# nju-ee/MODE-2022

Hardware: AMD Instinct MI355X
Metric: ERP stereo pairs/sec (512x1024, 192 disp) fwd+bwd (higher is better)
Workload: dtype fp32 storage/accumulate; products: 2xfp16 split (22-bit, per-tensor 2^k scale, 3 MFMAs) in the stride-1 3x3x3 / spherical / 3x3 layers incl. gradients (DESIGN 3u/3v); 3xbf16 split (24-bit, 6 MFMAs) in the stride-2 / transposed 3x3x3 layers and the polar spherical tiles (3j-3l); fp32 MFMA in the 32->; 1 GPU; ModeDisparity(192,Sphere,1024x512 Cassini) fwd+bwd+Adam step, batch 2/GPU (BASELINE configs[2]); global_batch=2, conv_arith=bf16x6, init=recipe state, seed 1 (tests/golden/recipe.py), parallelism=dp1

## Files before the change

### mode-2022_amd/csrc/sphere_conv_win.hip

```cpp
#include <algorithm>
#include <cstring>
#include <vector>

#include "common.h"
#include "bn_internal.h"
#include "sphere_internal.h"
#include "sphere_tap.h"

namespace {

typedef float f32x16 __attribute__((ext_vector_type(16)));
typedef float f32x32 __attribute__((ext_vector_type(32)));

constexpr int RB = 2;
constexpr int TH = 32 * RB;
constexpr int TW = 4;
constexpr int WC = 8;
constexpr int CCH = 8;
constexpr int KT = 9;
constexpr int MTW = 4;
constexpr int NTHREADS = 64 * TW * RB;
constexpr int SROWS = NTHREADS / WC;
constexpr int WR_SMALL = TH + 17, WR_MID = TH + 81;
constexpr int WR_PIPE_MAX = 5 * SROWS;

struct WinDims {
  int B, Ci, H, W, Co, G;
  int Cig, Cog;
  int NCH;
  int MG;
  int wr;
  int wrap_pipe;
  int sh, sw;
  int accumulate;
};

__host__ __device__ constexpr int chan_pitch(int wr) {
  return WC * wr + ((32 - (WC * wr) % 64) + 64) % 64;
}

__device__ __forceinline__ f32x16 mfma32(float a, float b, f32x16 c) {
  return __builtin_amdgcn_mfma_f32_32x32x2f32(a, b, c, 0, 0, 0);
}

__global__ void pack_w_win(const float* __restrict__ w, float* __restrict__ wp, WinDims d, int fold, mode_bn_epilogue bn) {
  const long long total = (long long)d.G * d.MG * d.NCH * KT * MTW * 64 * 4;
  if (fold && blockIdx.x == 0)
    for (int o = threadIdx.x; o < d.Co; o += blockDim.x) wp[total + o] = fold_shift(bn, o);
  for (long long idx = (long long)blockIdx.x * blockDim.x + threadIdx.x; idx < total; idx += (long long)gridDim.x * blockDim.x) {
    const int s = (int)(idx & 3);
    const int lane = (int)((idx >> 2) & 63);
    long long r = idx >> 8;
    const int m = (int)(r % MTW);
    r /= MTW;
    const int tap = (int)(r % KT);
    r /= KT;
    const int ch = (int)(r % d.NCH);
    r /= d.NCH;
    const int mg = (int)(r % d.MG);
    const int g = (int)(r / d.MG);
    const int co = mg * 128 + m * 32 + (lane & 31);
    const int c = ch * CCH + 2 * s + (lane >> 5);
    float v = 0.f;
    if (co < d.Cog && c < d.Cig) {
      v = w[((long long)(g * d.Cog + co) * d.Cig + c) * KT + tap];
      if (fold) v *= fold_scale(bn, g * d.Cog + co);
    }
    wp[idx] = v;
  }
}

template <int WR_T, bool PIPE, int NRB, int NPH, bool EPI>
__device__ __forceinline__ void fwd_tile(const float* __restrict__ x, const float* __restrict__ pos, const float4* __restrict__ wp,
                                         float* __restrict__ y, const WinDims& d, int h0, int w0, int rbase, int cbase, float* smem,
                                         const Epi& epi) {
  const int WRP = WR_T > 0 ? WR_T : d.wr;
  const int CP = chan_pitch(WRP);
  const int bufsz = CCH * CP;

  const int b = blockIdx.y;
  const int g = blockIdx.z / d.MG, mg = blockIdx.z % d.MG;
  const int tid = threadIdx.x;
  const int wave = tid >> 6, lane = tid & 63;
  const int half = lane >> 5;
  const int h = h0 + (wave / TW) * 32 + (lane & 31), w = w0 + (wave % TW);
  const bool pix_ok = h < d.H && w < d.W;
  const long long HW = (long long)d.H * d.W;

// ... 168 lines not shown
          for (int r = 0; r < 16; ++r) {
            const int co = min(m * 32 + (r & 3) + 8 * (r >> 2) + 4 * half, cmax - 1);
            res[r] = epi.add[(yb - y) + (long long)co * HW];
          }
        }
        __builtin_amdgcn_sched_barrier(0);
      }
      auto emit = [&](int r) {
        const int co = m * 32 + (r & 3) + 8 * (r >> 2) + 4 * half;
        if (EPI) {
          const float v = (acc[m][r] + shv[r]) + res[r];
          yb[(long long)co * HW] = epi.relu ? relu_nan(v) : v;
        } else {
          yb[(long long)co * HW] = acc[m][r];
        }
      };
      if (m * 32 + 32 <= cmax) {
#pragma unroll
        for (int r = 0; r < 16; ++r) emit(r);
      } else {
#pragma unroll
        for (int r = 0; r < 16; ++r)
          if (m * 32 + (r & 3) + 8 * (r >> 2) + 4 * half < cmax) emit(r);
      }
      if (EPI) __builtin_amdgcn_sched_barrier(0);
    }
  }
}

template <bool EPI>
__global__ __launch_bounds__(NTHREADS) void sphere_fwd_win_kernel(const float* __restrict__ x, const float* __restrict__ pos,
                                                                   const float4* __restrict__ wp, float* __restrict__ y, WinDims d,
                                                                   const int4* __restrict__ tiles, Epi epi) {
  extern __shared__ __attribute__((aligned(16))) float smem[];
  const int4 t = tiles[blockIdx.x];
  const int cls = t.w >> 16, cbase = t.w & 0xffff;
  if (cls == 0)
    fwd_tile<WR_SMALL, true, (WR_SMALL + SROWS - 1) / SROWS, 1, EPI>(x, pos, wp, y, d, t.x, t.y, t.z, cbase, smem, epi);
  else if (cls == 1)
    fwd_tile<WR_MID, true, (WR_MID + SROWS - 1) / SROWS, 2, EPI>(x, pos, wp, y, d, t.x, t.y, t.z, cbase, smem, epi);
  else
    fwd_tile<0, true, WR_PIPE_MAX / SROWS, 4, EPI>(x, pos, wp, y, d, t.x, t.y, t.z, cbase, smem, epi);
}

template <bool EPI>
__global__ __launch_bounds__(NTHREADS) void sphere_fwd_win_tall_kernel(const float* __restrict__ x, const float* __restrict__ pos,
                                                                        const float4* __restrict__ wp, float* __restrict__ y,
                                                                        WinDims d, const int4* __restrict__ tiles, Epi epi) {
  extern __shared__ __attribute__((aligned(16))) float smem[];
  const int4 t = tiles[blockIdx.x];
  fwd_tile<0, false, 1, 1, EPI>(x, pos, wp, y, d, t.x, t.y, t.z, t.w & 0xffff, smem, epi);
}

constexpr int BW_CG = 32;
constexpr int BW_TH = 32;
constexpr int BW_WR = BW_TH + 17;
constexpr int BW_CP = WC * BW_WR + 1;
constexpr int BW_GP = BW_TH + 1;
constexpr int BW_SLOTS = KT;
constexpr int BW_XW = BW_CG * BW_CP + BW_WR + 8;
constexpr int BW_COLBUF = 128 * BW_GP;
constexpr int BW_LDS_FLOATS = 2 * BW_XW + 2 * BW_COLBUF;
constexpr int BW_NXW = BW_CG / TW;
constexpr int BW_NREC = KT * BW_TH;

template <int WRP, int CP>
__device__ __forceinline__ void bww_column(const float* cb, const float* xw, const float4 rw, const int ro, const float4 rw8,
                                           const int ro8, f32x32 (&accp)[2], f32x32 (&acc8p)[2], int wave_u, int j, int half) {
  const float* ap = cb + (half * 32 + j) * BW_GP;
  const float* xb = xw + j * CP;
  auto load_x = [&](int o, float (&raw)[4]) {
    const float* p = xb + o;
    raw[0] = p[0];
    raw[1] = p[WRP];
    raw[2] = p[1];
    raw[3] = p[WRP + 1];
  };
  auto bcast = [&](float v, int px) { return __builtin_bit_cast(float, __builtin_amdgcn_readlane(__builtin_bit_cast(int, v), px)); };
  auto combine = [&](const float4& w, int px, const float (&raw)[4]) {
    return __builtin_fmaf(bcast(w.w, px), raw[3],
                          __builtin_fmaf(bcast(w.z, px), raw[2], __builtin_fmaf(bcast(w.y, px), raw[1], bcast(w.x, px) * raw[0])));
  };
  {
    float raw[2][4], a[3][2];
#pragma unroll
    for (int p0 = 0; p0 < 2; ++p0) {
      load_x(__builtin_amdgcn_readlane(ro, p0), raw[p0]);
      a[p0][0] = ap[p0];
      a[p0][1] = ap[64 * BW_GP + p0];
    }
    float bv = combine(rw, 0, raw[0]);
#pragma unroll
    for (int px = 0; px < BW_TH; ++px) {
      const int c3 = px % 3, n3 = (px + 2) % 3;
      float bv_next = 0.f;
      if (px + 1 < BW_TH) bv_next = combine(rw, px + 1, raw[(px + 1) & 1]);
      if (px + 2 < BW_TH) {
        load_x(__builtin_amdgcn_readlane(ro, px + 2), raw[px & 1]);
        a[n3][0] = ap[px + 2];
        a[n3][1] = ap[64 * BW_GP + px + 2];
      }
      __builtin_amdgcn_sched_barrier(0);
      accp[0] = __builtin_amdgcn_mfma_f32_32x32x1f32(a[c3][0], bv, accp[0], 0, 0, 0);
      accp[1] = __builtin_amdgcn_mfma_f32_32x32x1f32(a[c3][1], bv, accp[1], 0, 0, 0);
      __builtin_amdgcn_sched_barrier(0);
      bv = bv_next;
    }
  }
  {
    float raw[4][4], a[4][2];
#pragma unroll
    for (int i = 0; i < BW_TH / 8; ++i) {
      const int px = wave_u + 8 * i;
      load_x(__builtin_amdgcn_readlane(ro8, px), raw[i]);
      a[i][0] = ap[px];
      a[i][1] = ap[64 * BW_GP + px];
    }
// ... 272 lines not shown
    const float* pp = part + ((((long long)z * NCG + cg) * BW_SLOTS + k) * 128 + row) * BW_CG + cl;
    float a0 = 0.f, a1 = 0.f, a2 = 0.f, a3 = 0.f;
    int e = 0;
    for (; e + 3 < S; e += 4) {
      a0 += pp[(long long)e * stride];
      a1 += pp[(long long)(e + 1) * stride];
      a2 += pp[(long long)(e + 2) * stride];
      a3 += pp[(long long)(e + 3) * stride];
    }
    for (; e < S; ++e) a0 += pp[(long long)e * stride];
    const float sum = (a0 + a1) + (a2 + a3);
    gw[((long long)(g * d.Cog + ol) * d.Cig + c) * KT + k] += sum;
  }
}

bool halves_fit(const float* pos_host, int H, int W, int KK, int h0, int w0, int rbase, int cbase) {
  const long long HW = (long long)H * W;
  for (int hf = 0; hf < 2; ++hf) {
    const int rb = (rbase + hf * BW_TH) % H;
    for (int k = 0; k < KK; ++k)
      for (int h = h0 + hf * BW_TH; h < std::min(h0 + (hf + 1) * BW_TH, H); ++h)
        for (int w = w0; w < std::min(w0 + TW, W); ++w) {
          int r0, c0;
          float4 wt;
          const long long idx = (long long)h * W + w;
          if (!mode::tap_record_fixed(pos_host[(2 * k) * HW + idx], pos_host[(2 * k + 1) * HW + idx], H, W, r0, c0, wt)) continue;
          if (wt.x == 0.f && wt.y == 0.f && wt.z == 0.f && wt.w == 0.f) continue;
          const int lr = ((r0 - rb) % H + H) % H;
          if (lr + 1 >= BW_WR || c0 - cbase < 0 || c0 - cbase + 1 >= WC) return false;
        }
  }
  return true;
}

int bww_win_splits(const WinDims& d, int ntiles) {
  const int T = ntiles * 2 * d.B;
  const int wgs_per_slice = mode::cdiv(d.Cig, BW_CG) * d.G * d.MG;
  const int per = std::max(1, mode::cdiv((long long)T * wgs_per_slice, kNumCU));
  return std::max(1, mode::cdiv(T, per));
}


constexpr int SP_CCH = 16;
constexpr int SP_CP = chan_pitch(WR_SMALL);
constexpr int SP_WIN = SP_CCH * SP_CP;
constexpr int SP_WIN_FLOATS = ((2 * SP_WIN + WR_SMALL + 8 + 3) / 4) * 4;
constexpr int SP_OP = 8 * 3 * 64;
constexpr size_t SP_LDS_BYTES = (size_t)SP_WIN_FLOATS * sizeof(float) + 2 * (size_t)SP_OP * sizeof(uint4);
constexpr size_t SP3_LDS_BYTES = SP_LDS_BYTES + (size_t)SP_OP * sizeof(uint4);
static_assert(SP3_LDS_BYTES <= 160 * 1024, "windows + three operand buffers must fit the 160 KB of a CU");

typedef __bf16 sp_bf16x8 __attribute__((ext_vector_type(8)));
typedef __bf16 sp_bf16x2 __attribute__((ext_vector_type(2)));
typedef float sp_f32x2 __attribute__((ext_vector_type(2)));

__device__ __forceinline__ uint32_t sp_pack2(float a, float b) {
  const sp_f32x2 v = {a, b};
  return __builtin_bit_cast(uint32_t, __builtin_convertvector(v, sp_bf16x2));
}
__device__ __forceinline__ void sp_split2(float a, float b, uint32_t& p1, uint32_t& p2, uint32_t& p3) {
  p1 = sp_pack2(a, b);
  float ra = a - __builtin_bit_cast(float, p1 << 16), rb = b - __builtin_bit_cast(float, p1 & 0xffff0000u);
  asm("" : "+v"(ra), "+v"(rb));
  p2 = sp_pack2(ra, rb);
  float sa = ra - __builtin_bit_cast(float, p2 << 16), sb = rb - __builtin_bit_cast(float, p2 & 0xffff0000u);
  asm("" : "+v"(sa), "+v"(sb));
  p3 = sp_pack2(sa, sb);
}
__device__ __forceinline__ f32x16 sp_mfma(uint4 a, uint4 b, f32x16 c) {
  return __builtin_amdgcn_mfma_f32_32x32x16_bf16(__builtin_bit_cast(sp_bf16x8, a), __builtin_bit_cast(sp_bf16x8, b), c, 0, 0, 0);
}
__device__ __forceinline__ void sp_lds_barrier() { asm volatile("s_waitcnt lgkmcnt(0)\n\ts_barrier" ::: "memory"); }

typedef _Float16 sp_f16x2 __attribute__((ext_vector_type(2)));
typedef _Float16 sp_f16x8 __attribute__((ext_vector_type(8)));
__device__ __forceinline__ float sp_f16_scale_of(float m) {
  const unsigned e = min(max((__builtin_bit_cast(unsigned, m) >> 23) & 0xffu, 64u), 254u);
  return m == 0.f ? 1.f : __builtin_bit_cast(float, (268u - e) << 23);
}
__device__ __forceinline__ void sp_split2_f16(float a, float b, uint32_t& p1, uint32_t& p2) {
  const sp_f32x2 v = {a, b};
  const sp_f16x2 h1 = __builtin_convertvector(v, sp_f16x2);
  p1 = __builtin_bit_cast(uint32_t, h1);
  float ra, rb;
  asm("v_fma_mix_f32 %0, 1.0, %3, -%2 op_sel_hi:[0,0,1]\n\t"
      "v_fma_mix_f32 %1, 1.0, %4, -%2 op_sel:[0,0,1] op_sel_hi:[0,0,1]"
      : "=&v"(ra), "=&v"(rb)
      : "v"(p1), "v"(a), "v"(b));
  const sp_f32x2 r = {ra, rb};
  p2 = __builtin_bit_cast(uint32_t, __builtin_convertvector(r, sp_f16x2));
}
__device__ __forceinline__ f32x16 sp_mfma_f16(uint4 a, uint4 b, f32x16 c) {
  return __builtin_amdgcn_mfma_f32_32x32x16_f16(__builtin_bit_cast(sp_f16x8, a), __builtin_bit_cast(sp_f16x8, b), c, 0, 0, 0);
}

template <bool F16>
__global__ void pack_w_win_split(const float* __restrict__ w, uint4* __restrict__ wps, WinDims d, int NCH16, int fold, mode_bn_epilogue bn,
                                 const float* __restrict__ amax_w) {
  const float sw = F16 ? sp_f16_scale_of(mode::absmax_load(amax_w)) : 1.f;
  const long long total = (long long)d.G * d.MG * NCH16 * KT * MTW * 64;
  for (long long idx = (long long)blockIdx.x * blockDim.x + threadIdx.x; idx < total; idx += (long long)gridDim.x * blockDim.x) {
    const int lane = (int)(idx & 63);
    long long r = idx >> 6;
    const int m = (int)(r % MTW);
    r /= MTW;
    const int tap = (int)(r % KT);
    r /= KT;
    const int ch = (int)(r % NCH16);
    r /= NCH16;
    const int mg = (int)(r % d.MG);
    const int g = (int)(r / d.MG);
    const int co = mg * 128 + m * 32 + (lane & 31);
    float v[8];
#pragma unroll
    for (int j = 0; j < 8; ++j) {
      const int c = ch * SP_CCH + 8 * (lane >> 5) + j;
      v[j] = 0.f;
      if (co < d.Cog && c < d.Cig) {
        v[j] = w[((long long)(g * d.Cog + co) * d.Cig + c) * KT + tap];
        if (fold) v[j] *= fold_scale(bn, g * d.Cog + co);
        if (F16) v[j] *= sw;
      }
    }
    uint32_t q1[4], q2[4], q3[4];
#pragma unroll
    for (int j = 0; j < 4; ++j) {
      if constexpr (F16) {
        sp_split2_f16(v[2 * j], v[2 * j + 1], q1[j], q2[j]);
        q3[j] = 0u;
      } else {
        sp_split2(v[2 * j], v[2 * j + 1], q1[j], q2[j], q3[j]);
      }
    }
    uint4* dst = wps + (idx - lane) * 3 + lane;
    dst[0] = make_uint4(q1[0], q1[1], q1[2], q1[3]);
    dst[64] = make_uint4(q2[0], q2[1], q2[2], q2[3]);
    dst[128] = make_uint4(q3[0], q3[1], q3[2], q3[3]);
  }
}

constexpr int TP = 5;

template <bool F16>
__global__ void pack_w_win_split_tall(const float* __restrict__ w, uint4* __restrict__ wpt, WinDims d, int fold, mode_bn_epilogue bn,
                                      const float* __restrict__ amax_w) {
  const float sw = F16 ? sp_f16_scale_of(mode::absmax_load(amax_w)) : 1.f;
  const long long total = (long long)d.G * d.MG * d.NCH * TP * MTW * 64;
// ... 811 lines not shown
  }
#undef MODE_SB
  MODE_STAMP(2)

  const int hh = h0 + (wave / TW) * 32 + (lane & 31);
  const int cmax = d.Cog - mg * 128;
  float shv[16];
  if (EPI) {
#pragma unroll
    for (int r = 0; r < 16; ++r) shv[r] = epi.shift[g * d.Cog + mg * 128 + min(m * 32 + (r & 3) + 8 * (r >> 2) + 4 * half, cmax - 1)];
  }
  const bool full_m = m * 32 + 32 <= cmax;
#pragma unroll
  for (int gi = 0; gi < 4; ++gi) {
    const int ww = w0 + gi;
    if (hh < d.H && ww < d.W) {
      float* yb = y + ((long long)b * d.Co + (long long)g * d.Cog + (long long)mg * 128) * HW + (long long)hh * d.sh + (long long)ww * d.sw;
      float res[16];
      if (EPI) {
#pragma unroll
        for (int r = 0; r < 16; ++r) res[r] = 0.f;
        if (epi.add) {
#pragma unroll
          for (int r = 0; r < 16; ++r) {
            const int co = min(m * 32 + (r & 3) + 8 * (r >> 2) + 4 * half, cmax - 1);
            res[r] = epi.add[(yb - y) + (long long)co * HW];
          }
        }
        __builtin_amdgcn_sched_barrier(0);
      }
      auto emit = [&](int r) {
        const int co = m * 32 + (r & 3) + 8 * (r >> 2) + 4 * half;
        if (EPI) {
          const float v = (acc[gi][r] + shv[r]) + res[r];
          yb[(long long)co * HW] = epi.relu ? relu_nan(v) : v;
        } else {
          yb[(long long)co * HW] = F16 ? acc[gi][r] * unscale : acc[gi][r];
        }
      };
      if (full_m) {
#pragma unroll
        for (int r = 0; r < 16; ++r) emit(r);
      } else {
#pragma unroll
        for (int r = 0; r < 16; ++r)
          if (m * 32 + (r & 3) + 8 * (r >> 2) + 4 * half < cmax) emit(r);
      }
      if (EPI) __builtin_amdgcn_sched_barrier(0);
    }
  }
  MODE_STAMP(3)
}

constexpr int BS_GP = 20;
constexpr int BS_GYB = 3 * 128 * BS_GP;
constexpr int BS_SCRP = 17;
constexpr int BS_SCR = 32 * BS_SCRP;
constexpr int BS_X2 = ((2 * BW_XW + 3) / 4) * 4;
constexpr int BS_LDS_DWORDS = BS_X2 + BS_GYB + 8 * BS_SCR;

template <bool F16>
__global__ __launch_bounds__(NTHREADS) void sphere_bww_split_kernel(const float* __restrict__ gy, const float* __restrict__ x,
                                                                     float* __restrict__ part, WinDims d, const int4* __restrict__ tiles,
                                                                     const float4* __restrict__ rec_w, const int* __restrict__ rec_off,
                                                                     int ntiles, int S, const float* __restrict__ amax_g,
                                                                     const float* __restrict__ amax_x) {
  extern __shared__ __attribute__((aligned(16))) float smem[];
  float sg = 1.f, sx = 1.f, unscale = 1.f;
  if (F16) {
    sg = sp_f16_scale_of(mode::absmax_load(amax_g));
    sx = sp_f16_scale_of(mode::absmax_load(amax_x));
    unscale = (1.f / sg) * (1.f / sx);
  }
  constexpr int NPC = F16 ? 2 : 3;
  uint32_t* gyb = reinterpret_cast<uint32_t*>(smem + BS_X2);
  constexpr int WRP = BW_WR, CP = BW_CP;
  const int s = blockIdx.x, cg = blockIdx.y;
  const int g = blockIdx.z / d.MG, mg = blockIdx.z % d.MG;
  const int tid = threadIdx.x;
  const int wave = tid >> 6, lane = tid & 63;
  const int j = lane & 31, half = lane >> 5;
  float* scr = smem + BS_X2 + BS_GYB + wave * BS_SCR;
  const long long HW = (long long)d.H * d.W;
  const int T = ntiles * 2 * d.B;
  const int NCG = gridDim.y;

  f32x16 acc[4], acc8;
#pragma unroll
  for (int r = 0; r < 16; ++r) {
    acc[0][r] = acc[1][r] = acc[2][r] = acc[3][r] = 0.f;
    acc8[r] = 0.f;
  }
  for (int i = tid; i < BS_LDS_DWORDS; i += NTHREADS) smem[i] = 0.f;

  const int omax = d.Cog - mg * 128;
  const int cmax = d.Cig - cg * BW_CG;
  const int sh = half, sq = j >> 3, sp8 = j & 7;
  const int ks8 = wave >> 2, m8 = wave & 3;

  struct Item {
    int b, ti, hf, h0, w0, rbase, cbase;
  };
  auto item_of = [&](int t) {
    Item it;
    it.b = t / (ntiles * 2);
    const int r = t - it.b * ntiles * 2;
    it.ti = r >> 1;
// ... 861 lines not shown
                                                     const int32_t* tiles, int n_small, int n_mid, int n_wrap, const float* rec_w,
                                                     const int32_t* rec_off, const int32_t* rest_pixels, int n_rest_pixels,
                                                     const int32_t* pitems, const float* prec_w, const int32_t* prec_off,
                                                     int n_polar_items, int B, int Ci, int H, int W, int Co, int Kh, int Kw, int groups,
                                                     const float* gy_t, const float* x_t, mode_stream_t stream) {
  return bwd_weight_win_impl(gy, pos, x, gw, workspace, tiles, n_small, n_mid, n_wrap, rec_w, rec_off, rest_pixels, n_rest_pixels, pitems,
                             prec_w, prec_off, n_polar_items, B, Ci, H, W, Co, Kh, Kw, groups, gy_t, x_t, stream, 1);
}

extern "C" int mode_sphere_conv_bwd_weight_win_split_f16(const float* gy, const float* pos, const float* x, const float* amax_g,
                                                         const float* amax_x, float* gw, float* workspace, const int32_t* tiles, int n_small,
                                                         int n_mid, int n_wrap, const float* rec_w, const int32_t* rec_off,
                                                         const int32_t* rest_pixels, int n_rest_pixels, const int32_t* pitems,
                                                         const float* prec_w, const int32_t* prec_off, int n_polar_items, int B, int Ci, int H,
                                                         int W, int Co, int Kh, int Kw, int groups, const float* gy_t, const float* x_t,
                                                         mode_stream_t stream) {
  MODE_REQUIRE(amax_g && amax_x, MODE_ERR_BAD_ARG, "mode_sphere_conv_bwd_weight_win_split_f16: null maximum");
  return bwd_weight_win_impl(gy, pos, x, gw, workspace, tiles, n_small, n_mid, n_wrap, rec_w, rec_off, rest_pixels, n_rest_pixels, pitems,
                             prec_w, prec_off, n_polar_items, B, Ci, H, W, Co, Kh, Kw, groups, gy_t, x_t, stream, 1, amax_g, amax_x);
}

static int bwd_weight_win_impl(const float* gy, const float* pos, const float* x, float* gw, float* workspace, const int32_t* tiles,
                               int n_small, int n_mid, int n_wrap, const float* rec_w, const int32_t* rec_off, const int32_t* rest_pixels,
                               int n_rest_pixels, const int32_t* pitems, const float* prec_w, const int32_t* prec_off, int n_polar_items,
                               int B, int Ci, int H, int W, int Co, int Kh, int Kw, int groups, const float* gy_t, const float* x_t,
                               mode_stream_t stream, int split, const float* amax_g, const float* amax_x) {
  WinDims d;
  int rc = make_win_dims(d, B, Ci, H, W, Co, Kh, Kw, groups, "mode_sphere_conv_bwd_weight_win");
  MODE_REQUIRE((amax_g == nullptr) == (amax_x == nullptr), MODE_ERR_BAD_ARG, "mode_sphere_conv_bwd_weight_win: both operand maxima, or neither");
  if (rc != MODE_OK) return rc;
  MODE_REQUIRE((gy_t == nullptr) == (x_t == nullptr), MODE_ERR_BAD_ARG, "mode_sphere_conv_bwd_weight_win: gy_t and x_t come together");
  if (gy_t) {
    d.sh = 1;
    d.sw = H;
  }
  MODE_REQUIRE(n_small >= 0 && n_mid >= 0 && n_wrap >= 0 && n_rest_pixels >= 0 && n_polar_items >= 0 &&
                   (size_t)n_small + n_mid + n_wrap == mode_sphere_plan_max_tiles(H, W),
               MODE_ERR_BAD_ARG, "mode_sphere_conv_bwd_weight_win: the plan must cover every tile");
  if (B == 0) return MODE_OK;
  MODE_REQUIRE(((gy && x) || (gy_t && n_rest_pixels == 0)) && pos && gw && workspace && tiles && (n_rest_pixels == 0 || rest_pixels) &&
                   (n_small == 0 || (rec_w && rec_off)) &&
                   (n_polar_items == 0 || (pitems && prec_w && prec_off)),
               MODE_ERR_BAD_ARG, "mode_sphere_conv_bwd_weight_win: null pointer");
  hipStream_t st = mode::as_stream(stream);
  const int NCG = mode::cdiv(d.Cig, BW_CG);
  const size_t slice = (size_t)d.G * d.MG * NCG * BW_SLOTS * 128 * BW_CG * sizeof(float);
  const float* gys = gy_t ? gy_t : gy;
  const float* xs = x_t ? x_t : x;
  int S = 0;
  if (n_small > 0) {
    S = bww_win_splits(d, n_small);
    if (split) {
      const size_t lds = (size_t)BS_LDS_DWORDS * sizeof(float);
      if (amax_g) {
        rc = mode::allow_lds(sphere_bww_split_kernel<true>, lds, "mode_sphere_conv_bwd_weight_win_split");
        if (rc != MODE_OK) return rc;
        hipLaunchKernelGGL(sphere_bww_split_kernel<true>, dim3(S, NCG, d.G * d.MG), dim3(NTHREADS), lds, st, gys, xs, workspace, d,
                           reinterpret_cast<const int4*>(tiles) + n_wrap + n_mid, reinterpret_cast<const float4*>(rec_w), rec_off, n_small, S,
                           amax_g, amax_x);
      } else {
        rc = mode::allow_lds(sphere_bww_split_kernel<false>, lds, "mode_sphere_conv_bwd_weight_win_split");
        if (rc != MODE_OK) return rc;
        hipLaunchKernelGGL(sphere_bww_split_kernel<false>, dim3(S, NCG, d.G * d.MG), dim3(NTHREADS), lds, st, gys, xs, workspace, d,
                           reinterpret_cast<const int4*>(tiles) + n_wrap + n_mid, reinterpret_cast<const float4*>(rec_w), rec_off, n_small, S,
                           amax_g, amax_x);
      }
    } else {
      const size_t lds = (size_t)BW_LDS_FLOATS * sizeof(float);
      rc = mode::allow_lds(sphere_bww_win_kernel, lds, "mode_sphere_conv_bwd_weight_win");
      if (rc != MODE_OK) return rc;
      hipLaunchKernelGGL(sphere_bww_win_kernel, dim3(S, NCG, d.G * d.MG), dim3(NTHREADS), lds, st, gys, xs, workspace, d,
                         reinterpret_cast<const int4*>(tiles) + n_wrap + n_mid, reinterpret_cast<const float4*>(rec_w), rec_off, n_small, S);
    }
    rc = mode::check_launch("mode_sphere_conv_bwd_weight_win");
    if (rc != MODE_OK) return rc;
  }
  int Sp = 0;
  if (n_polar_items > 0) {
    Sp = bww_polar_splits(d, n_polar_items);
    if (split) {
      const size_t lds = (size_t)BQ_LDS_DWORDS * sizeof(float);
      rc = mode::allow_lds(sphere_bww_polar_split_kernel, lds, "mode_sphere_conv_bwd_weight_win_split");
      if (rc != MODE_OK) return rc;
      hipLaunchKernelGGL(sphere_bww_polar_split_kernel, dim3(Sp, NCG, d.G * d.MG), dim3(NTHREADS), lds, st, gys, xs, workspace, d, pitems,
                         reinterpret_cast<const float4*>(prec_w), prec_off, n_polar_items, Sp, S);
    } else {
      const size_t lds = (size_t)BP_LDS_FLOATS * sizeof(float);
      rc = mode::allow_lds(sphere_bww_polar_kernel, lds, "mode_sphere_conv_bwd_weight_win");
      if (rc != MODE_OK) return rc;
      hipLaunchKernelGGL(sphere_bww_polar_kernel, dim3(Sp, NCG, d.G * d.MG), dim3(NTHREADS), lds, st, gys, xs, workspace, d, pitems,
                         reinterpret_cast<const float4*>(prec_w), prec_off, n_polar_items, Sp, S);
    }
    rc = mode::check_launch("mode_sphere_conv_bwd_weight_win(polar)");
    if (rc != MODE_OK) return rc;
  }
  if (S + Sp > 0) {
    const long long n = (long long)d.G * d.MG * NCG * KT * 128 * BW_CG;
    hipLaunchKernelGGL(reduce_gw_win, dim3(mode::cdiv(n, 256)), dim3(256), 0, st, workspace, gw, d, S + Sp, NCG);
    rc = mode::check_launch("mode_sphere_conv_bwd_weight_win(reduce)");
    if (rc != MODE_OK) return rc;
  }
  if (n_rest_pixels > 0)
    return mode::sphere_bwd_weight_general(gy, pos, x, gw, reinterpret_cast<float*>(reinterpret_cast<char*>(workspace) + slice * (S + Sp)), B,
                                           Ci, H, W, Co, Kh, Kw, 1, 1, H, W, groups, rest_pixels, n_rest_pixels, st,
                                           "mode_sphere_conv_bwd_weight_win(rest)");
  return MODE_OK;
}
// ... 665 lines not shown
```

### mode-2022_amd/mode_hip/build.py

```python
import os
import subprocess
import sys
from concurrent.futures import ThreadPoolExecutor

HERE = os.path.dirname(os.path.abspath(__file__))
PKG = os.path.dirname(HERE)
ROOT = os.path.dirname(PKG)
CSRC = os.path.join(PKG, 'csrc')
INCLUDE = os.path.join(ROOT, 'include')
OBJ = os.path.join(CSRC, 'obj')
LIB = os.path.join(HERE, 'libmode_hip.so')

HIPCC = os.environ.get('HIPCC', '/opt/rocm/bin/hipcc')
FLAGS = ['--offload-arch=gfx950', '-O3', '-std=c++17', '-fPIC', '-munsafe-fp-atomics', '-Wall', '-Wno-unused-function',
         '-I' + INCLUDE, '-I' + CSRC]
FLAGS += ['-D' + d for d in os.environ.get('MODE_HIP_DEFINES', '').split()]


def sources():
  return sorted(os.path.join(CSRC, f) for f in os.listdir(CSRC) if f.endswith('.hip'))


def _deps_mtime():
  hs = [os.path.join(CSRC, f) for f in os.listdir(CSRC) if f.endswith('.h')]
  hs += [os.path.join(INCLUDE, f) for f in os.listdir(INCLUDE)]
  hs.append(os.path.abspath(__file__))
  return max(os.path.getmtime(h) for h in hs)


FILE_FLAGS = {
    'conv3d_split.hip': ['-fno-slp-vectorize'],
    'conv2d_split.hip': ['-fno-slp-vectorize'],
    'conv3d_split_wgrad.hip': ['-fno-slp-vectorize'],
    'conv2d_split_wgrad.hip': ['-fno-slp-vectorize'],
}


def _flags_of(src):
  return FLAGS + FILE_FLAGS.get(os.path.basename(src), [])


def _flags_hash(src):
  import hashlib
  return hashlib.sha256('\0'.join([HIPCC] + _flags_of(src)).encode()).hexdigest()


def _stamp(obj):
  return obj + '.flags'


def _compile(src, force):
  obj = os.path.join(OBJ, os.path.basename(src)[:-4] + '.o')
  want = _flags_hash(src)
  try:
    with open(_stamp(obj)) as f:
      have = f.read().strip()
  except OSError:
    have = None
  if (not force and have == want and os.path.exists(obj) and
      os.path.getmtime(obj) > max(os.path.getmtime(src), _deps_mtime())):
    return obj, False
  cmd = [HIPCC] + _flags_of(src) + ['-c', src, '-o', obj]
  r = subprocess.run(cmd, capture_output=True, text=True)
  if r.returncode != 0:
    raise RuntimeError('hipcc failed: %s\n%s\n%s' % (' '.join(cmd), r.stdout, r.stderr))
  if r.stderr.strip():
    sys.stderr.write(r.stderr)
  with open(_stamp(obj), 'w') as f:
    f.write(want)
  return obj, True


def build(force=False, verbose=True):
  os.makedirs(OBJ, exist_ok=True)
  srcs = sources()
  with ThreadPoolExecutor(max_workers=min(8, len(srcs))) as ex:
    results = list(ex.map(lambda s: _compile(s, force), srcs))
  objs = [o for o, _ in results]
  if force or any(c for _, c in results) or not os.path.exists(LIB):
    cmd = [HIPCC, '--offload-arch=gfx950', '-shared', '-fPIC', '-o', LIB] + objs
    r = subprocess.run(cmd, capture_output=True, text=True)
    if r.returncode != 0:
      raise RuntimeError('link failed: %s\n%s\n%s' % (' '.join(cmd), r.stdout, r.stderr))
    if verbose:
      print('built', LIB)
  elif verbose:
    print('up to date', LIB)
# ... 6 lines not shown
```

Measured before the change: 37.58 pairs/s.

## Add dedicated fp16-split sphere weight-gradient kernel with transposed LDS reads

Adds a new kernel for the spherical conv weight gradient on the fp16 2x-split path. It double-buffers the x windows and prefetches gy columns and tap records one step ahead. The sampled B operand goes through per-wave LDS images read with ds_read_tr16_b64, and scheduling group barriers interleave MFMAs with the VALU and LDS work. Shared definitions move to a new header, and the old split kernel stays as the fallback when 32-bit offsets would overflow. The new kernel brings more LDS use, register pressure and complexity, plus a risk in the unsigned offset arithmetic.

```diff
diff --git a/mode-2022_amd/csrc/sphere_bww_f16.hip b/mode-2022_amd/csrc/sphere_bww_f16.hip
--- /dev/null
+++ b/mode-2022_amd/csrc/sphere_bww_f16.hip
@@ -0,0 +1,364 @@
+#include "common.h"
+#include "bn_internal.h"
+#include "sphere_win.h"
+
+namespace mode {
+namespace win {
+namespace {
+
+constexpr int BF_X2 = ((2 * BW_XW + 3) / 4) * 4;
+constexpr int BF_GYB = 2 * 128 * BS_GP;
+constexpr int BF_IMG = 2 * 16 * 16;
+constexpr int BF_OWN = 8 * BF_IMG;
+constexpr int BF_T8 = 2 * 2 * BF_IMG;
+constexpr int BF_LDS_DWORDS = BF_X2 + BF_GYB + BF_OWN + BF_T8;
+static_assert(BF_LDS_DWORDS * 4 <= 160 * 1024, "the LDS of one CU");
+
+typedef short s16x4 __attribute__((ext_vector_type(4)));
+typedef __attribute__((address_space(3))) s16x4 lds_s16x4;
+
+template <typename T>
+__device__ __forceinline__ T ld_off(const T* base, uint32_t byte_off) {
+  return *reinterpret_cast<const T*>(reinterpret_cast<const char*>(base) + byte_off);
+}
+__device__ __forceinline__ uint2 tr_read(const uint32_t* p) {
+  return __builtin_bit_cast(uint2, __builtin_amdgcn_ds_read_tr16_b64_v4i16((lds_s16x4*)(p)));
+}
+
+__global__ __launch_bounds__(NTHREADS) void sphere_bww_f16_kernel(const float* __restrict__ gy, const float* __restrict__ x,
+                                                                  float* __restrict__ part, WinDims d, const int4* __restrict__ tiles,
+                                                                  const float4* __restrict__ rec_w, const int* __restrict__ rec_off,
+                                                                  int ntiles, int S, const float* __restrict__ amax_g,
+                                                                  const float* __restrict__ amax_x) {
+  extern __shared__ __attribute__((aligned(16))) float smem[];
+  const float sg = sp_f16_scale_of(absmax_load(amax_g));
+  const float sx = sp_f16_scale_of(absmax_load(amax_x));
+  const float unscale = (1.f / sg) * (1.f / sx);
+  uint32_t* const gyb = reinterpret_cast<uint32_t*>(smem + BF_X2);
+  uint32_t* const own = gyb + BF_GYB;
+  uint32_t* const t8 = own + BF_OWN;
+  constexpr int WRP = BW_WR, CP = BW_CP;
+  const int s = blockIdx.x, cg = blockIdx.y;
+  const int g = blockIdx.z / d.MG, mg = blockIdx.z % d.MG;
+  const int tid = threadIdx.x, lane = tid & 63;
+  const int wave = __builtin_amdgcn_readfirstlane(tid >> 6);
+  const int j = lane & 31, half = lane >> 5;
+  const int T = ntiles * 2 * d.B;
+  const int NCG = gridDim.y;
+  const int omax = d.Cog - mg * 128, cmax = d.Cig - cg * BW_CG;
+  const int ks8 = wave >> 2, m8 = wave & 3;
+  const uint32_t HW = (uint32_t)d.H * (uint32_t)d.W, HW4 = HW * 4u;
+
+  f32x16 acc[4], acc8;
+#pragma unroll
+  for (int r = 0; r < 16; ++r) {
+    acc[0][r] = acc[1][r] = acc[2][r] = acc[3][r] = 0.f;
+    acc8[r] = 0.f;
+  }
+  for (int i = tid; i < BF_LDS_DWORDS; i += NTHREADS) smem[i] = 0.f;
+
+  const int px0 = 8 * half + (lane & 7), sq = (lane >> 3) & 3;
+  const uint32_t rl_own = (uint32_t)(wave * BW_TH + px0), rl_t8 = (uint32_t)(8 * BW_TH + 16 * ks8 + px0);
+  float* const xsmp0 = smem + 8 * sq * CP;
+  float* const xsmp8 = smem + (8 * sq + 2 * m8) * CP;
+  uint32_t* const own_w = own + wave * BF_IMG + px0 * 16 + 4 * sq;
+  uint32_t* const t8_w = t8 + ks8 * BF_IMG + px0 * 16 + 4 * sq + m8;
+  const int trow = 8 * half + ((lane & 15) >> 2);
+  const int toff = trow * 16 + 8 * ((lane >> 4) & 1) + 2 * (lane & 3);
+  const uint32_t* const own_r = own + wave * BF_IMG + toff;
+  const uint32_t* const t8_r = t8 + ks8 * BF_IMG + toff;
+  const int ga_off = j * BS_GP + 4 * half;
+  const int gpp = lane & 15, gol = lane >> 4;
+  uint32_t* const gy_w = gyb + (16 * wave + gol) * BS_GP + gpp;
+  uint32_t go_lane[4];
+  unsigned go_ok = 0;
+#pragma unroll
+  for (int u = 0; u < 4; ++u) {
+    const int o = 16 * wave + 4 * u + gol;
+    go_lane[u] = (uint32_t)min(o, omax - 1) * HW4;
+    go_ok |= (o < omax ? 1u : 0u) << u;
+  }
+  const int xcol = d.sh == 1 ? tid >> 6 : tid & (WC - 1), xrow = d.sh == 1 ? tid & 63 : tid >> 3;
+  const bool xrow_ok = xrow < WRP;
+  float* const xw_w = smem + xcol * WRP + (xrow_ok ? xrow : 0);
+
+  const float* const gyz = gy + ((long long)g * d.Cog + (long long)mg * 128) * HW;
+  const float* const xz = x + ((long long)g * d.Cig + (long long)cg * BW_CG) * HW;
+
+  struct Item {
+    const float* gyb;
+    const float* xb;
+    const float4* rw;
+    const int* ro;
+    int w0;
+    uint32_t gy_lane0;
+    uint32_t gy_lane1;
+    uint32_t x_lane;
+    unsigned ok;
+  };
+  auto item_of = [&](int t) {
+    Item it;
+    const int b = t / (ntiles * 2);
+    const int r = t - b * ntiles * 2;
+    const int ti = r >> 1, hf = r & 1;
+    const int4 tl = tiles[ti];
+    const int h0 = tl.x + hf * BW_TH, rbase = (tl.z + hf * BW_TH) % d.H, cbase = tl.w & 0xffff;
+    it.w0 = tl.y;
+    it.gyb = gyz + (long long)b * d.Co * HW;
+    it.xb = xz + (long long)b * d.Ci * HW;
+    const long long rb = ((long long)ti * 2 + hf) * TW * BW_NREC;
+    it.rw = rec_w + rb;
+    it.ro = rec_off + rb;
+    const int h = h0 + 2 * gpp;
+    const bool ok0 = h < d.H, ok1 = h + 1 < d.H;
+    it.gy_lane0 = ok0 ? (uint32_t)h * (uint32_t)d.sh * 4u : 0u;
+    it.gy_lane1 = ok1 ? (uint32_t)(h + 1) * (uint32_t)d.sh * 4u : it.gy_lane0;
+    const bool xok = xrow_ok && cbase + xcol < d.W;
+    const int grow = (rbase + (xrow_ok ? xrow : 0)) % d.H;
+    it.x_lane = xok ? ((uint32_t)grow * (uint32_t)d.sh + (uint32_t)(cbase + xcol) * (uint32_t)d.sw) * 4u : 0u;
+    it.ok = (ok0 ? 1u : 0u) | (ok1 ? 2u : 0u) | (xok ? 4u : 0u);
+    return it;
+  };
+
+  auto issue_xw = [&](const Item& it, int part, float (&v)[BW_NXW]) {
+    int cm = cmax;
+    asm volatile("" : "+s"(cm));
+#pragma unroll
+    for (int c = 0; c < BW_NXW; ++c) v[c] = ld_off(it.xb, it.x_lane + (uint32_t)min(part * BW_NXW + c, cm - 1) * HW4);
+  };
+  auto commit_xw = [&](float* xwdst, const Item& it, int part, const float (&v)[BW_NXW]) {
+    if (xrow_ok) {
+#pragma unroll
+      for (int c = 0; c < BW_NXW; ++c)
+        xwdst[(part * BW_NXW + c) * CP] = ((it.ok & 4u) && part * BW_NXW + c < cmax) ? v[c] : 0.f;
+    }
+  };
+  struct GyPF {
+    float g0[4], g1[4];
+    unsigned ok;
+  };
+  auto issue_gy = [&](const Item& it, int wc, GyPF& pf) {
+    const int w = it.w0 + wc;
+    const bool wok = w < d.W;
+    const float* col = it.gyb + (wok ? (long long)w * d.sw : 0);
+#pragma unroll
+    for (int u = 0; u < 4; ++u) {
+      pf.g0[u] = ld_off(col, go_lane[u] + it.gy_lane0);
+      pf.g1[u] = ld_off(col, go_lane[u] + it.gy_lane1);
+    }
+    const unsigned pix = wok ? (it.ok & 3u) : 0u;
+    pf.ok = 0;
+#pragma unroll
+    for (int u = 0; u < 4; ++u) pf.ok |= ((go_ok >> u & 1u) ? pix : 0u) << (2 * u);
+  };
+  auto commit_col = [&](uint32_t* dst, const GyPF& pf) {
+#pragma unroll
+    for (int u = 0; u < 4; ++u) {
+      const float a = (pf.ok >> (2 * u) & 1u) ? pf.g0[u] : 0.f, b2 = (pf.ok >> (2 * u + 1) & 1u) ? pf.g1[u] : 0.f;
+      uint32_t p1, p2;
+      sp_split2_f16(a * sg, b2 * sg, p1, p2);
+      dst[4 * u * BS_GP] = p1;
+      dst[128 * BS_GP + 4 * u * BS_GP] = p2;
+    }
+  };
+  struct Rec {
+    float4 w0, w1, w8;
+    int o0, o1, o8;
+  };
+  auto issue_rec = [&](const Item& it, int wc, Rec& rc) {
+    const float4* rw = it.rw + wc * BW_NREC;
+    const int* ro = it.ro + wc * BW_NREC;
+    rc.w0 = ld_off(rw, rl_own * 16u);
+    rc.o0 = ld_off(ro, rl_own * 4u);
+    rc.w1 = ld_off(rw + 16, rl_own * 16u);
+    rc.o1 = ld_off(ro + 16, rl_own * 4u);
+    rc.w8 = ld_off(rw, rl_t8 * 16u);
+    rc.o8 = ld_off(ro, rl_t8 * 4u);
+  };
+  auto scaled = [&](const float4 w) { return make_float4(w.x * sx, w.y * sx, w.z * sx, w.w * sx); };
+  auto sample_own = [&](int xbuf, const float4 w4_, int ro) {
+    const float* xb = xsmp0 + xbuf * BW_XW + ro;
+    float r_[8][4];
+#pragma unroll
+    for (int c = 0; c < 8; ++c) {
+      const float* q = xb + c * CP;
+      r_[c][0] = q[0];
+      r_[c][1] = q[WRP];
+      r_[c][2] = q[1];
+      r_[c][3] = q[WRP + 1];
+    }
+    __builtin_amdgcn_sched_barrier(0);
+    const float4 w4 = scaled(w4_);
+    float v[8];
+#pragma unroll
+    for (int c = 0; c < 8; ++c) {
+      v[c] = __builtin_fmaf(w4.w, r_[c][3], __builtin_fmaf(w4.z, r_[c][2], __builtin_fmaf(w4.y, r_[c][1], w4.x * r_[c][0])));
+      asm("" : "+v"(v[c]));
+    }
+    uint32_t h[4], l[4];
+#pragma unroll
+    for (int i = 0; i < 4; ++i) sp_split2_f16(v[2 * i], v[2 * i + 1], h[i], l[i]);
+    uint4* dst = reinterpret_cast<uint4*>(own_w);
+    dst[0] = make_uint4(h[0], h[1], h[2], h[3]);
+    dst[16 * 16 / 4] = make_uint4(l[0], l[1], l[2], l[3]);
+  };
+  auto sample_t8 = [&](int xbuf, const float4 w4_, int ro, int par) {
+    const float* xb = xsmp8 + xbuf * BW_XW + ro;
+    float r_[2][4];
+#pragma unroll
+    for (int c = 0; c < 2; ++c) {
+      const float* q = xb + c * CP;
+      r_[c][0] = q[0];
+      r_[c][1] = q[WRP];
+      r_[c][2] = q[1];
+      r_[c][3] = q[WRP + 1];
+    }
+    const float4 w4 = scaled(w4_);
+    float v[2];
+#pragma unroll
+    for (int c = 0; c < 2; ++c) {
+      v[c] = __builtin_fmaf(w4.w, r_[c][3], __builtin_fmaf(w4.z, r_[c][2], __builtin_fmaf(w4.y, r_[c][1], w4.x * r_[c][0])));
+      asm("" : "+v"(v[c]));
+    }
+    uint32_t h, l;
+    sp_split2_f16(v[0], v[1], h, l);
+    uint32_t* dst = t8_w + par * 2 * BF_IMG;
+    dst[0] = h;
+    dst[16 * 16] = l;
+  };
+  auto read_b = [&](const uint32_t* r, int p) {
+    const uint2 lo = tr_read(r + p * 256), hi = tr_read(r + p * 256 + 64);
+    return make_uint4(lo.x, lo.y, hi.x, hi.y);
+  };
+  auto load_a = [&](int ks, uint4 (&a)[4][2]) {
+#pragma unroll
+    for (int m = 0; m < 4; ++m) {
+      const uint4* ga = reinterpret_cast<const uint4*>(gyb + ga_off + m * 32 * BS_GP + 8 * ks);
+      a[m][0] = ga[0];
+      a[m][1] = ga[128 * BS_GP / 4];
+    }
+  };
+  auto mma12 = [&](const uint4 (&a)[4][2], const uint4 (&b)[2]) {
+#pragma unroll
+    for (int m = 0; m < 4; ++m) acc[m] = sp_mfma_f16(a[m][1], b[0], acc[m]);
+#pragma unroll
+    for (int m = 0; m < 4; ++m) acc[m] = sp_mfma_f16(a[m][0], b[1], acc[m]);
+#pragma unroll
+    for (int m = 0; m < 4; ++m) acc[m] = sp_mfma_f16(a[m][0], b[0], acc[m]);
+  };
+#define MODE_BF_SPREAD(nv, nl)                           \
+  _Pragma("unroll") for (int i_ = 0; i_ < 12; ++i_) {    \
+    __builtin_amdgcn_sched_group_barrier(0x008, 1, 0);   \
+    __builtin_amdgcn_sched_group_barrier(0x002, nv, 0);  \
+    __builtin_amdgcn_sched_group_barrier(0x100, nl, 0);  \
+  }                                                      \
+  __builtin_amdgcn_sched_barrier(0);
+
+  Item cur = item_of(s);
+  GyPF gpf[2];
+  Rec rec;
+  __syncthreads();
+#pragma unroll
+  for (int part = 0; part < TW; ++part) {
+    float v[BW_NXW];
+    issue_xw(cur, part, v);
+    commit_xw(xw_w, cur, part, v);
+  }
+  issue_gy(cur, 0, gpf[0]);
+  issue_rec(cur, 0, rec);
+  commit_col(gy_w, gpf[0]);
+  issue_gy(cur, 1, gpf[1]);
+  __syncthreads();
+  sample_own(0, rec.w0, rec.o0);
+  sample_t8(0, rec.w8, rec.o8, 0);
+  __syncthreads();
+
+  int xbuf = 0;
+  for (int t = s; t < T; t += S) {
+    const bool more_items = t + S < T;
+    const Item nxt = item_of(more_items ? t + S : t);
+#pragma unroll
+    for (int wc = 0; wc < TW; ++wc) {
+      float xv[2][BW_NXW];
+      if (wc < 3) issue_xw(nxt, wc, xv[0]);
+      if (wc == 2) issue_xw(nxt, 3, xv[1]);
+      const float4 w1 = rec.w1;
+      const int o1 = rec.o1;
+      issue_rec(wc == TW - 1 ? nxt : cur, wc == TW - 1 ? 0 : wc + 1, rec);
+      issue_gy(wc < 2 ? cur : nxt, wc < 2 ? wc + 2 : wc - 2, gpf[wc & 1]);
+      __builtin_amdgcn_sched_barrier(0);
+
+      uint4 a[4][2], b[2];
+      b[0] = read_b(own_r, 0);
+      b[1] = read_b(own_r, 1);
+      load_a(0, a);
+      sample_own(xbuf, w1, o1);
+      mma12(a, b);
+      MODE_BF_SPREAD(5, 4)
+      b[0] = read_b(own_r, 0);
+      b[1] = read_b(own_r, 1);
+      load_a(1, a);
+      const int nbuf = wc == TW - 1 ? xbuf ^ 1 : xbuf;
+      sample_own(nbuf, rec.w0, rec.o0);
+      sample_t8(nbuf, rec.w8, rec.o8, (wc + 1) & 1);
+      mma12(a, b);
+      MODE_BF_SPREAD(6, 4)
+      {
+        const uint32_t* t8r = t8_r + (wc & 1) * 2 * BF_IMG;
+        const uint4 b0 = read_b(t8r, 0), b1 = read_b(t8r, 1);
+        const uint4* ga = reinterpret_cast<const uint4*>(gyb + ga_off + m8 * 32 * BS_GP + 8 * ks8);
+        const uint4 a1 = ga[0], a2 = ga[128 * BS_GP / 4];
+        acc8 = sp_mfma_f16(a2, b0, acc8);
+        acc8 = sp_mfma_f16(a1, b1, acc8);
+        acc8 = sp_mfma_f16(a1, b0, acc8);
+      }
+      float* xwn = xw_w + (xbuf ^ 1) * BW_XW;
+      if (wc < 3) commit_xw(xwn, nxt, wc, xv[0]);
+      if (wc == 2) commit_xw(xwn, nxt, 3, xv[1]);
+      __syncthreads();
+      commit_col(gy_w, gpf[(wc + 1) & 1]);
+      __syncthreads();
+    }
+    cur = nxt;
+    xbuf ^= 1;
+  }
+#undef MODE_BF_SPREAD
+
+  float* pb = part + ((((long long)s * gridDim.z + blockIdx.z) * NCG + cg) * BW_SLOTS) * (128 * BW_CG);
+#pragma unroll
+  for (int m = 0; m < 4; ++m)
+#pragma unroll
+    for (int r = 0; r < 16; ++r) {
+      const int o = m * 32 + (r & 3) + 8 * (r >> 2) + 4 * half;
+      pb[((long long)wave * 128 + o) * BW_CG + j] = acc[m][r] * unscale;
+    }
+  float* red = smem;
+  if (wave < 4) {
+#pragma unroll
+    for (int r = 0; r < 16; ++r) red[(m8 * 32 + (r & 3) + 8 * (r >> 2) + 4 * half) * BW_CG + j] = acc8[r] * unscale;
+  }
+  __syncthreads();
+  if (wave >= 4) {
+#pragma unroll
+    for (int r = 0; r < 16; ++r) red[(m8 * 32 + (r & 3) + 8 * (r >> 2) + 4 * half) * BW_CG + j] += acc8[r] * unscale;
+  }
+  __syncthreads();
+  for (int i = tid; i < 128 * BW_CG; i += NTHREADS) pb[(long long)8 * 128 * BW_CG + i] = red[i];
+}
+
+}
+
+bool bww_f16_fits(const WinDims& d) { return (long long)d.H * d.W * 128 * sizeof(float) < (1ll << 32); }
+
+int launch_bww_f16(const float* gy, const float* x, float* part, const WinDims& d, const int4* tiles, const float4* rec_w,
+                   const int* rec_off, int ntiles, int S, int NCG, const float* amax_g, const float* amax_x, hipStream_t st) {
+  const size_t lds = (size_t)BF_LDS_DWORDS * sizeof(float);
+  const int rc = allow_lds(sphere_bww_f16_kernel, lds, "mode_sphere_conv_bwd_weight_win_split_f16");
+  if (rc != MODE_OK) return rc;
+  hipLaunchKernelGGL(sphere_bww_f16_kernel, dim3(S, NCG, d.G * d.MG), dim3(NTHREADS), lds, st, gy, x, part, d, tiles, rec_w, rec_off,
+                     ntiles, S, amax_g, amax_x);
+  return MODE_OK;
+}
+
+}
+}
diff --git a/mode-2022_amd/csrc/sphere_conv_win.hip b/mode-2022_amd/csrc/sphere_conv_win.hip
--- a/mode-2022_amd/csrc/sphere_conv_win.hip
+++ b/mode-2022_amd/csrc/sphere_conv_win.hip
@@ -6,34 +6,20 @@
 #include "bn_internal.h"
 #include "sphere_internal.h"
 #include "sphere_tap.h"
+#include "sphere_win.h"
 
 namespace {
 
-typedef float f32x16 __attribute__((ext_vector_type(16)));
+using namespace mode::win;
+
 typedef float f32x32 __attribute__((ext_vector_type(32)));
 
-constexpr int RB = 2;
 constexpr int TH = 32 * RB;
-constexpr int TW = 4;
-constexpr int WC = 8;
 constexpr int CCH = 8;
-constexpr int KT = 9;
 constexpr int MTW = 4;
-constexpr int NTHREADS = 64 * TW * RB;
 constexpr int SROWS = NTHREADS / WC;
 constexpr int WR_SMALL = TH + 17, WR_MID = TH + 81;
 constexpr int WR_PIPE_MAX = 5 * SROWS;
-
-struct WinDims {
-  int B, Ci, H, W, Co, G;
-  int Cig, Cog;
-  int NCH;
-  int MG;
-  int wr;
-  int wrap_pipe;
-  int sh, sw;
-  int accumulate;
-};
 
 __host__ __device__ constexpr int chan_pitch(int wr) {
   return WC * wr + ((32 - (WC * wr) % 64) + 64) % 64;
@@ -308,17 +294,9 @@
   fwd_tile<0, false, 1, 1, EPI>(x, pos, wp, y, d, t.x, t.y, t.z, t.w & 0xffff, smem, epi);
 }
 
-constexpr int BW_CG = 32;
-constexpr int BW_TH = 32;
-constexpr int BW_WR = BW_TH + 17;
-constexpr int BW_CP = WC * BW_WR + 1;
 constexpr int BW_GP = BW_TH + 1;
-constexpr int BW_SLOTS = KT;
-constexpr int BW_XW = BW_CG * BW_CP + BW_WR + 8;
 constexpr int BW_COLBUF = 128 * BW_GP;
 constexpr int BW_LDS_FLOATS = 2 * BW_XW + 2 * BW_COLBUF;
-constexpr int BW_NXW = BW_CG / TW;
-constexpr int BW_NREC = KT * BW_TH;
 
 template <int WRP, int CP>
 __device__ __forceinline__ void bww_column(const float* cb, const float* xw, const float4 rw, const int ro, const float4 rw8,
@@ -697,7 +675,6 @@
 
 typedef __bf16 sp_bf16x8 __attribute__((ext_vector_type(8)));
 typedef __bf16 sp_bf16x2 __attribute__((ext_vector_type(2)));
-typedef float sp_f32x2 __attribute__((ext_vector_type(2)));
 
 __device__ __forceinline__ uint32_t sp_pack2(float a, float b) {
   const sp_f32x2 v = {a, b};
@@ -717,27 +694,6 @@
 }
 __device__ __forceinline__ void sp_lds_barrier() { asm volatile("s_waitcnt lgkmcnt(0)\n\ts_barrier" ::: "memory"); }
 
-typedef _Float16 sp_f16x2 __attribute__((ext_vector_type(2)));
-typedef _Float16 sp_f16x8 __attribute__((ext_vector_type(8)));
-__device__ __forceinline__ float sp_f16_scale_of(float m) {
-  const unsigned e = min(max((__builtin_bit_cast(unsigned, m) >> 23) & 0xffu, 64u), 254u);
-  return m == 0.f ? 1.f : __builtin_bit_cast(float, (268u - e) << 23);
-}
-__device__ __forceinline__ void sp_split2_f16(float a, float b, uint32_t& p1, uint32_t& p2) {
-  const sp_f32x2 v = {a, b};
-  const sp_f16x2 h1 = __builtin_convertvector(v, sp_f16x2);
-  p1 = __builtin_bit_cast(uint32_t, h1);
-  float ra, rb;
-  asm("v_fma_mix_f32 %0, 1.0, %3, -%2 op_sel_hi:[0,0,1]\n\t"
-      "v_fma_mix_f32 %1, 1.0, %4, -%2 op_sel:[0,0,1] op_sel_hi:[0,0,1]"
-      : "=&v"(ra), "=&v"(rb)
-      : "v"(p1), "v"(a), "v"(b));
-  const sp_f32x2 r = {ra, rb};
-  p2 = __builtin_bit_cast(uint32_t, __builtin_convertvector(r, sp_f16x2));
-}
-__device__ __forceinline__ f32x16 sp_mfma_f16(uint4 a, uint4 b, f32x16 c) {
-  return __builtin_amdgcn_mfma_f32_32x32x16_f16(__builtin_bit_cast(sp_f16x8, a), __builtin_bit_cast(sp_f16x8, b), c, 0, 0, 0);
-}
 
 template <bool F16>
 __global__ void pack_w_win_split(const float* __restrict__ w, uint4* __restrict__ wps, WinDims d, int NCH16, int fold, mode_bn_epilogue bn,
@@ -1655,7 +1611,6 @@
   MODE_STAMP(3)
 }
 
-constexpr int BS_GP = 20;
 constexpr int BS_GYB = 3 * 128 * BS_GP;
 constexpr int BS_SCRP = 17;
 constexpr int BS_SCR = 32 * BS_SCRP;
@@ -2623,7 +2578,11 @@
     S = bww_win_splits(d, n_small);
     if (split) {
       const size_t lds = (size_t)BS_LDS_DWORDS * sizeof(float);
-      if (amax_g) {
+      if (amax_g && bww_f16_fits(d)) {
+        rc = launch_bww_f16(gys, xs, workspace, d, reinterpret_cast<const int4*>(tiles) + n_wrap + n_mid, reinterpret_cast<const float4*>(rec_w),
+                            rec_off, n_small, S, NCG, amax_g, amax_x, st);
+        if (rc != MODE_OK) return rc;
+      } else if (amax_g) {
         rc = mode::allow_lds(sphere_bww_split_kernel<true>, lds, "mode_sphere_conv_bwd_weight_win_split");
         if (rc != MODE_OK) return rc;
         hipLaunchKernelGGL(sphere_bww_split_kernel<true>, dim3(S, NCG, d.G * d.MG), dim3(NTHREADS), lds, st, gys, xs, workspace, d,
diff --git a/mode-2022_amd/csrc/sphere_win.h b/mode-2022_amd/csrc/sphere_win.h
--- /dev/null
+++ b/mode-2022_amd/csrc/sphere_win.h
@@ -0,0 +1,67 @@
+#pragma once
+#include <hip/hip_runtime.h>
+
+#include <cstdint>
+
+namespace mode {
+namespace win {
+
+typedef float f32x16 __attribute__((ext_vector_type(16)));
+
+constexpr int RB = 2;
+constexpr int TW = 4;
+constexpr int WC = 8;
+constexpr int KT = 9;
+constexpr int NTHREADS = 64 * TW * RB;
+
+struct WinDims {
+  int B, Ci, H, W, Co, G;
+  int Cig, Cog;
+  int NCH;
+  int MG;
+  int wr;
+  int wrap_pipe;
+  int sh, sw;
+  int accumulate;
+};
+
+constexpr int BW_CG = 32;
+constexpr int BW_TH = 32;
+constexpr int BW_WR = BW_TH + 17;
+constexpr int BW_CP = WC * BW_WR + 1;
+constexpr int BW_SLOTS = KT;
+constexpr int BW_XW = BW_CG * BW_CP + BW_WR + 8;
+constexpr int BW_NXW = BW_CG / TW;
+constexpr int BW_NREC = KT * BW_TH;
+constexpr int BS_GP = 20;
+
+typedef float sp_f32x2 __attribute__((ext_vector_type(2)));
+
+typedef _Float16 sp_f16x2 __attribute__((ext_vector_type(2)));
+typedef _Float16 sp_f16x8 __attribute__((ext_vector_type(8)));
+__device__ __forceinline__ float sp_f16_scale_of(float m) {
+  const unsigned e = min(max((__builtin_bit_cast(unsigned, m) >> 23) & 0xffu, 64u), 254u);
+  return m == 0.f ? 1.f : __builtin_bit_cast(float, (268u - e) << 23);
+}
+__device__ __forceinline__ void sp_split2_f16(float a, float b, uint32_t& p1, uint32_t& p2) {
+  const sp_f32x2 v = {a, b};
+  const sp_f16x2 h1 = __builtin_convertvector(v, sp_f16x2);
+  p1 = __builtin_bit_cast(uint32_t, h1);
+  float ra, rb;
+  asm("v_fma_mix_f32 %0, 1.0, %3, -%2 op_sel_hi:[0,0,1]\n\t"
+      "v_fma_mix_f32 %1, 1.0, %4, -%2 op_sel:[0,0,1] op_sel_hi:[0,0,1]"
+      : "=&v"(ra), "=&v"(rb)
+      : "v"(p1), "v"(a), "v"(b));
+  const sp_f32x2 r = {ra, rb};
+  p2 = __builtin_bit_cast(uint32_t, __builtin_convertvector(r, sp_f16x2));
+}
+__device__ __forceinline__ f32x16 sp_mfma_f16(uint4 a, uint4 b, f32x16 c) {
+  return __builtin_amdgcn_mfma_f32_32x32x16_f16(__builtin_bit_cast(sp_f16x8, a), __builtin_bit_cast(sp_f16x8, b), c, 0, 0, 0);
+}
+
+bool bww_f16_fits(const WinDims& d);
+int launch_bww_f16(const float* gy, const float* x, float* part, const WinDims& d, const int4* tiles, const float4* rec_w,
+                   const int* rec_off, int ntiles, int S, int NCG, const float* amax_g, const float* amax_x, hipStream_t st);
+
+}
+}
diff --git a/mode-2022_amd/mode_hip/build.py b/mode-2022_amd/mode_hip/build.py
--- a/mode-2022_amd/mode_hip/build.py
+++ b/mode-2022_amd/mode_hip/build.py
@@ -33,6 +33,7 @@
     'conv2d_split.hip': ['-fno-slp-vectorize'],
     'conv3d_split_wgrad.hip': ['-fno-slp-vectorize'],
     'conv2d_split_wgrad.hip': ['-fno-slp-vectorize'],
+    'sphere_bww_f16.hip': ['-fno-slp-vectorize'],
 }
 
 
```

After: 37.81 pairs/s, median of 6. Within noise of the previous version (+0.6%).
